# xxlong0/ESTDepth

Measured on AMD Instinct MI355X. Metric: depth frames/sec (seq_len=5, 480x640, D=64), higher is better.
Workload: dtype f32

## Files before the change

### estdepth_amd/build.py

```python
import os
import subprocess
import sys
from concurrent.futures import ThreadPoolExecutor

HERE = os.path.dirname(os.path.abspath(__file__))
ROOT = os.path.dirname(HERE)
CSRC = os.path.join(HERE, "csrc")
OUT_DIR = os.path.join(HERE, "lib")
OBJ_DIR = os.path.join(OUT_DIR, "obj" + os.environ.get("ESTD_LIB_SUFFIX", ""))
LIB = os.path.join(OUT_DIR, "libestd_hip%s.so" % os.environ.get("ESTD_LIB_SUFFIX", ""))
SOURCES = ["conv3d_mfma.hip", "conv3d_wino2.hip", "conv3d_wino3.hip", "conv3d_xout.hip", "conv3d_wino2_c16.hip", "conv2d_mfma.hip", "conv2d_wino2.hip",
           "plane_sweep.hip", "est_fusion.hip", "refine2d.hip", "conv1x1.hip", "conv2d_taps.hip", "tsdf.hip", "tsdf_raycast.hip",
           "depth_consistency.hip", "cloud_nn.hip"]
AB_SOURCES = ["conv3d_wino.hip", "conv3d_split_bf16.hip", "conv2d_wino.hip", "conv2d_split_bf16.hip", "conv3d_wino2x.hip"]
BUILD_AB = os.environ.get("ESTD_BUILD_AB", "0") == "1"
if BUILD_AB:
    SOURCES = SOURCES + AB_SOURCES
HEADERS = [os.path.join(ROOT, "include", "estd_hip.h"), os.path.join(CSRC, "estd_common.h")]
FLAGS = ["--offload-arch=gfx950", "-O3", "-std=c++17", "-fPIC",
         "-I" + os.path.join(ROOT, "include"), "-I" + CSRC] + (["-DESTD_BUILD_AB=1"] if BUILD_AB else [])
MODE_STAMP = os.path.join(OUT_DIR, ".build_mode" + os.environ.get("ESTD_LIB_SUFFIX", ""))


def _hipcc():
    for c in (os.environ.get("HIPCC"), "/opt/rocm/bin/hipcc", "hipcc"):
        if c and (os.path.isabs(c) and os.path.exists(c) or not os.path.isabs(c)):
            return c
    return "hipcc"


def _stale(target, deps):
    if not os.path.exists(target):
        return True
    t = os.path.getmtime(target)
    return any(os.path.getmtime(d) > t for d in deps)


def build(force=False, verbose=False):
    os.makedirs(OBJ_DIR, exist_ok=True)
    hipcc = _hipcc()
    mode = "ab" if BUILD_AB else "default"
    relink = (open(MODE_STAMP).read().strip() if os.path.exists(MODE_STAMP) else "default" if os.path.exists(LIB) else "") != mode
    jobs = []
    objs = []
    for src in SOURCES:
        s = os.path.join(CSRC, src)
        o = os.path.join(OBJ_DIR, src.replace(".hip", ".o"))
        objs.append(o)
        if force or _stale(o, [s] + HEADERS):
            cmd = [hipcc] + FLAGS + os.environ.get("ESTD_BUILD_DEFS", "").split() + (["-Rpass-analysis=kernel-resource-usage"] if verbose else []) + ["-c", s, "-o", o]
            jobs.append(cmd)

    def run(cmd):
        r = subprocess.run(cmd, capture_output=True, text=True)
        if r.returncode != 0:
            raise RuntimeError("hipcc failed: %s\n%s" % (" ".join(cmd), r.stderr))
        return r.stderr

    if jobs:
        with ThreadPoolExecutor(max_workers=len(jobs)) as ex:
            for log in ex.map(run, jobs):
                if verbose and log:
                    sys.stderr.write(log)
    if force or jobs or relink or _stale(LIB, objs):
        run([hipcc, "--offload-arch=gfx950", "-shared", "-fPIC"] + objs + ["-o", LIB])
    build_torch_ops(force=force or relink)
    open(MODE_STAMP, "w").write(mode)
    return LIB


TORCH_OPS_SRC = os.path.join(CSRC, "torch_ops.cpp")
TORCH_OPS_LIB = os.path.join(OUT_DIR, "libestd_torch_ops%s.so" % os.environ.get("ESTD_LIB_SUFFIX", ""))


def build_torch_ops(force=False):
    if not (force or _stale(TORCH_OPS_LIB, [TORCH_OPS_SRC, HEADERS[0], LIB])):
        return TORCH_OPS_LIB
    import torch
    from torch.utils import cpp_extension
    tlib = os.path.join(os.path.dirname(torch.__file__), "lib")
    cmd = [_hipcc(), "-O2", "-std=c++17", "-fPIC", "-shared", "-D__HIP_PLATFORM_AMD__=1", "-DUSE_ROCM=1", "-DHIPBLAS_V2",
           "-D_GLIBCXX_USE_CXX11_ABI=%d" % int(torch._C._GLIBCXX_USE_CXX11_ABI), "-I" + os.path.join(ROOT, "include")] \
        + (["-DESTD_BUILD_AB=1"] if BUILD_AB else [])
    cmd += ["-I" + p for p in cpp_extension.include_paths("cuda")]
    cmd += [TORCH_OPS_SRC, "-o", TORCH_OPS_LIB, "-L" + OUT_DIR, "-l:" + os.path.basename(LIB), "-L" + tlib,
            "-lc10", "-lc10_hip", "-ltorch_cpu", "-ltorch_hip", "-ltorch", "-Wl,-rpath,$ORIGIN", "-Wl,-rpath," + tlib]
    r = subprocess.run(cmd, capture_output=True, text=True)
    if r.returncode != 0:
        raise RuntimeError("hipcc failed: %s\n%s" % (" ".join(cmd), r.stderr[-4000:]))
    return TORCH_OPS_LIB


if __name__ == "__main__":
    print(build(force="--force" in sys.argv, verbose="--verbose" in sys.argv))
```

### estdepth_amd/csrc/conv2d_wino2.hip

```cpp
#include <hip/hip_runtime.h>
#include <stdint.h>
#include <stdlib.h>
#include <type_traits>

#include "estd_hip.h"
#include "estd_common.h"

#ifndef ESTD_C2W2ABL
#define ESTD_C2W2ABL 0
#endif

namespace {

typedef float f32x4 __attribute__((ext_vector_type(4)));
typedef float f32x2 __attribute__((ext_vector_type(2)));
typedef unsigned int u32x4 __attribute__((__vector_size__(16)));
constexpr unsigned OOB_OFFSET = 0xFFFFFF00u;

constexpr int TH = 8, TW = 16;
constexpr int TROWS = 16;
constexpr int NSTEP = 8;
#ifndef ESTD_C2W2_PFS
#define ESTD_C2W2_PFS 8
#endif
#ifndef ESTD_C2W2_WD
#define ESTD_C2W2_WD 2
#endif
#ifndef ESTD_C2W2_INLOOP
#define ESTD_C2W2_INLOOP 1
#endif
#ifndef ESTD_C2W2_INLOOP_PFS
#define ESTD_C2W2_INLOOP_PFS 4
#endif
#ifndef ESTD_C2W2_INLOOP_W0
#define ESTD_C2W2_INLOOP_W0 4
#endif
#ifndef ESTD_C2W2_SCHED
#define ESTD_C2W2_SCHED 2
#endif
#ifndef ESTD_C2W2_SPLIT
#define ESTD_C2W2_SPLIT 1
#endif
constexpr int WD = ESTD_C2W2_WD, WR = 4;

__device__ __forceinline__ float4 as_float4(u32x4 v) { float4 f; __builtin_memcpy(&f, &v, 16); return f; }
__device__ __forceinline__ u32x4 as_u32x4(float4 f) { u32x4 v; __builtin_memcpy(&v, &f, 16); return v; }
__device__ __forceinline__ float4 f4_sub(float4 a, float4 b) { return make_float4(a.x - b.x, a.y - b.y, a.z - b.z, a.w - b.w); }
__device__ __forceinline__ float4 f4_add(float4 a, float4 b) { return make_float4(a.x + b.x, a.y + b.y, a.z + b.z, a.w + b.w); }
__device__ __forceinline__ __amdgpu_buffer_rsrc_t make_rsrc(const float* base, size_t elems)
{
    return __builtin_amdgcn_make_buffer_rsrc(const_cast<float*>(base), 0, (int)(elems * 4), 0x00020000);
}
__device__ __forceinline__ void lds_barrier() { asm volatile("s_waitcnt lgkmcnt(0)\n\ts_barrier" ::: "memory"); }

template <int DIL>
__device__ __forceinline__ void wino2_rpp_nt(const estd_conv2d_desc& p, int tiles_w, int tiles_h, int total_items)
{
    constexpr int IN_H = TH + 2 * DIL, IN_W = TW + 2 * DIL;
    constexpr bool INLOOP = ESTD_C2W2_INLOOP != 0 && (DIL == 1 || ESTD_C2W2_INLOOP == 2);
    constexpr int PITCH = DIL == 1 ? IN_W + 1 : IN_W;
    constexpr int SLOT_BYTES = TROWS * PITCH * 128;
    constexpr int SH_BYTES = 4 * PITCH * 128;
    constexpr int LOADERS = IN_W * 8;
    auto lds_off = [](int row, int col, int chunk) { return (row * PITCH + col) * 128 + ((chunk ^ ((col >> 1) & 7)) << 4); };
    extern __shared__ __attribute__((aligned(16))) char smem[];

    const int tid = threadIdx.x;
    const int lane = tid & 63;
    const int wave = __builtin_amdgcn_readfirstlane(tid >> 6);
    const int rpp = wave >> 1, nt = wave & 1;
    const int g = lane >> 4, i = lane & 15;
    const int blk_rp = (i >= 4 && i < 12) ? 1 : 0;
    const int cb = i < 4 ? i : i < 12 ? i - 4 : i - 8;
    const int rp = 2 * rpp + blk_rp;
    const int row_a = DIL == 1 ? 2 * rp : (rp & 1) + 4 * (rp >> 1);
    const int col_b = DIL == 1 ? 2 * cb : (cb & 1) + 4 * (cb >> 1);
    const int H = p.H, W = p.W, Cin = p.cin, Cout = p.cout;
    const int nchunks = Cin >> 5;
    const int tiles_per_group = p.N * tiles_h * tiles_w;
    const int wlane = lane * 16 + nt * 1024;

    int u, u_end;
    {
        const int G = gridDim.x, bid = blockIdx.x;
        const int r = ((G & 7) == 0) ? (bid & 7) * (G >> 3) + (bid >> 3) : bid;
        u = (int)((long long)total_items * r / G);
        u_end = (int)((long long)total_items * (r + 1) / G);
    }
    if (u >= u_end) return;

    const size_t img_in = (size_t)H * W * Cin, img_out = (size_t)H * W * Cout;
    const bool loader = tid < LOADERS;
    const int lzx = tid >> 3, lc = tid & 7;
    const int wbase = loader ? lds_off(0, lzx, lc) : 0;

    int aoff[4];
#pragma unroll
    for (int q = 0; q < 4; ++q) aoff[q] = lds_off(rp, col_b + DIL * q, g);

    auto decode = [&](int item, int& grp, int& n, int& th0, int& tw0) {
        grp = item / tiles_per_group;
        int t = item - grp * tiles_per_group;
        const int twi = t % tiles_w; t /= tiles_w;
        const int thi = t % tiles_h; n = t / tiles_h;
        th0 = thi * TH; tw0 = twi * TW;
    };
    auto brick_offsets = [&](int th0, int tw0, unsigned (&voff)[IN_H], bool enable) {
        const int gx = tw0 - DIL + lzx;
        const bool colok = enable && loader && (unsigned)gx < (unsigned)W;
        const unsigned base = (unsigned)(gx * Cin + lc * 4) * 4u;
        const unsigned rowbytes = (unsigned)(W * Cin) * 4u;
#pragma unroll
        for (int zy = 0; zy < IN_H; ++zy) {
            const int gy = th0 - DIL + zy;
            const bool rowok = (unsigned)gy < (unsigned)H;
            voff[zy] = (colok && rowok) ? base + (unsigned)gy * rowbytes : OOB_OFFSET;
        }
    };

    int grp, n, th0, tw0;
    decode(u, grp, n, th0, tw0);
    unsigned voff[IN_H];
    brick_offsets(th0, tw0, voff, true);
    __amdgpu_buffer_rsrc_t rs_in = make_rsrc(p.in + (size_t)n * img_in, img_in);
    float4 pf[IN_H];
#pragma unroll
    for (int zy = 0; zy < IN_H; ++zy) pf[zy] = as_float4(__builtin_amdgcn_raw_buffer_load_b128(rs_in, voff[zy], 0, 0));

    const size_t wgrp_elems = (size_t)nchunks * NSTEP * 4 * 2 * 256;
    float4 bq[WR][4];
    {
        const __amdgpu_buffer_rsrc_t rs_w0 = make_rsrc(p.w_wino + (size_t)grp * wgrp_elems, wgrp_elems);
#pragma unroll
        for (int s = 0; s < WD; ++s)
#pragma unroll
            for (int sw = 0; sw < 4; ++sw) bq[s][sw] = as_float4(__builtin_amdgcn_raw_buffer_load_b128(rs_w0, wlane, (s * 4 + sw) * 2048, 0));
    }
    const float floor_b = p.relu_before_residual ? 0.f : ESTD_NO_FLOOR;
    const float floor_a = p.relu_after_residual ? 0.f : ESTD_NO_FLOOR;

    int k = 0;
    if (INLOOP) {
        if (loader && !(ESTD_C2W2ABL & 2)) {
#pragma unroll
            for (int w = 0; w < 4; ++w) {
                const int a = DIL == 1 ? 2 * w : (w & 1) + 4 * (w >> 1);
                const float4 d0 = pf[a], d1 = pf[a + DIL], d2 = pf[a + 2 * DIL], d3 = pf[a + 3 * DIL];
                *reinterpret_cast<float4*>(smem + wbase + (0 * 4 + w) * PITCH * 128) = f4_sub(d0, d2);
                *reinterpret_cast<float4*>(smem + wbase + (1 * 4 + w) * PITCH * 128) = f4_add(d1, d2);
                *reinterpret_cast<float4*>(smem + wbase + (2 * 4 + w) * PITCH * 128) = f4_sub(d2, d1);
                *reinterpret_cast<float4*>(smem + wbase + (3 * 4 + w) * PITCH * 128) = f4_sub(d1, d3);
            }
        }
    }
    while (true) {
        const __amdgpu_buffer_rsrc_t rs_w = make_rsrc(p.w_wino + (size_t)grp * wgrp_elems, wgrp_elems);
        const int cbase = grp * 32 + nt * 16 + 4 * g;
        const float4 sc4 = *reinterpret_cast<const float4*>(p.scale + cbase), sh4 = *reinterpret_cast<const float4*>(p.shift + cbase);
        f32x4 acc[4][4];

        const bool has_next_item = (u + 1 < u_end);
        int ngrp = grp, nn_ = n, nth0 = th0, ntw0 = tw0;
        if (has_next_item) decode(u + 1, ngrp, nn_, nth0, ntw0);
        const __amdgpu_buffer_rsrc_t rs_wni = make_rsrc(p.w_wino + (size_t)ngrp * wgrp_elems, wgrp_elems);

        auto write_rows = [&](char* slot, int w0, int w1) {
            if (loader && !(ESTD_C2W2ABL & 2)) {
#pragma unroll
                for (int w = 0; w < 4; ++w) {
                    if (w < w0 || w >= w1) continue;
                    const int a = DIL == 1 ? 2 * w : (w & 1) + 4 * (w >> 1);
                    const float4 d0 = pf[a], d1 = pf[a + DIL], d2 = pf[a + 2 * DIL], d3 = pf[a + 3 * DIL];
                    *reinterpret_cast<float4*>(slot + wbase + (0 * 4 + w) * PITCH * 128) = f4_sub(d0, d2);
                    *reinterpret_cast<float4*>(slot + wbase + (1 * 4 + w) * PITCH * 128) = f4_add(d1, d2);
                    *reinterpret_cast<float4*>(slot + wbase + (2 * 4 + w) * PITCH * 128) = f4_sub(d2, d1);
                    *reinterpret_cast<float4*>(slot + wbase + (3 * 4 + w) * PITCH * 128) = f4_sub(d1, d3);
                }
            }
        };
        auto write_row_sh = [&](char* slot, int w, int sh_) {
            if (loader && !(ESTD_C2W2ABL & 2)) {
                const int a = DIL == 1 ? 2 * w : (w & 1) + 4 * (w >> 1);
                const float4 d0 = pf[a], d1 = pf[a + DIL], d2 = pf[a + 2 * DIL], d3 = pf[a + 3 * DIL];
                const float4 v = sh_ == 0 ? f4_sub(d0, d2) : sh_ == 1 ? f4_add(d1, d2) : sh_ == 2 ? f4_sub(d2, d1) : f4_sub(d1, d3);
                *reinterpret_cast<float4*>(slot + wbase + (sh_ * 4 + w) * PITCH * 128) = v;
            }
        };
        auto chunk_body = [&](auto first_c, const int c) {
            constexpr bool FIRST = decltype(first_c)::value;
            const int sb = (k & 1) * SLOT_BYTES;
            char* slot = smem + sb;
            if (!INLOOP) write_rows(slot, 0, 4);
            lds_barrier();

            const bool last_chunk = (c + 1 == nchunks);
            int pf_soff = (c + 1) * 128;
            if (last_chunk) {
                brick_offsets(nth0, ntw0, voff, has_next_item);
                if (nn_ != n) rs_in = make_rsrc(p.in + (size_t)nn_ * img_in, img_in);
                pf_soff = 0;
            }
            const int wbase_q = c * NSTEP * 4;
            const __amdgpu_buffer_rsrc_t rs_wx = last_chunk ? rs_wni : rs_w;
            const int wnext_q = last_chunk ? 0 : wbase_q + NSTEP * 4;

            int ao[4];
#pragma unroll
            for (int q = 0; q < 4; ++q) ao[q] = aoff[q] + sb;
            auto load_rows = [&](int st, float4 (&Rr)[4]) {
#pragma unroll
                for (int q = 0; q < 4; ++q)
                    Rr[q] = *reinterpret_cast<const float4*>(smem + ((st & 1) ? (ao[q] ^ 64) : ao[q]) + (st >> 1) * SH_BYTES);
            };
            auto xform2 = [&](const float4 (&Rr)[4], int h, f32x2 (&o)[4]) {
                f32x2 r[4];
#pragma unroll
                for (int q = 0; q < 4; ++q) r[q] = h == 0 ? (f32x2){Rr[q].x, Rr[q].y} : (f32x2){Rr[q].z, Rr[q].w};
                if (ESTD_C2W2ABL & 128) { o[0] = r[0]; o[1] = r[1]; o[2] = r[2]; o[3] = r[3]; }
                else { o[0] = r[0] - r[2]; o[1] = r[1] + r[2]; o[2] = r[2] - r[1]; o[3] = r[1] - r[3]; }
            };
            f32x2 T[2][4];
            float4 R[4];
            load_rows(0, R);
            xform2(R, 0, T[0]);
            xform2(R, 1, T[1]);
            load_rows(1, R);
            __builtin_amdgcn_sched_barrier(0);

#pragma clang loop unroll(full)
            for (int st = 0; st < NSTEP; ++st) {
                const int sh = st >> 1;
                f32x2 Tn[2][4];
                if (ESTD_C2W2_SCHED == 2) {
                    constexpr int PFS = INLOOP ? ESTD_C2W2_INLOOP_PFS : ESTD_C2W2_PFS;
                    const int r0 = PFS != 8 ? (st < PFS ? st * IN_H / PFS : IN_H) : DIL == 1 ? (st == 0 ? 0 : st + 1) : (3 * st + 1) / 2;
                    const int r1 = PFS != 8 ? (st < PFS ? (st + 1) * IN_H / PFS : IN_H)
                                            : DIL == 1 ? ((st == 0 || st == NSTEP - 1) ? r0 + 2 : r0 + 1) : (3 * (st + 1) + 1) / 2;
                    const bool wr = INLOOP && st >= ESTD_C2W2_INLOOP_W0 && (!last_chunk || has_next_item);
                    constexpr int WN = NSTEP - ESTD_C2W2_INLOOP_W0;
                    static_assert(!INLOOP || WN == 4, "quarter schedule: one row pair of the next chunk per step");
#pragma unroll
                    for (int h = 0; h < 2; ++h) {
#pragma unroll
                        for (int e = 0; e < 2; ++e) {
                            const int qk = 2 * h + e;
                            if (!(ESTD_C2W2ABL & 8)) {
                                const int tgt = st + WD;
                                bq[tgt % WR][qk] = tgt < NSTEP
                                    ? as_float4(__builtin_amdgcn_raw_buffer_load_b128(rs_w, wlane, (wbase_q + tgt * 4 + qk) * 2048, 0))
                                    : as_float4(__builtin_amdgcn_raw_buffer_load_b128(rs_wx, wlane, (wnext_q + (tgt - NSTEP) * 4 + qk) * 2048, 0));
                            }
#pragma unroll
                            for (int r = r0 + (r1 - r0) * qk / 4; r < r0 + (r1 - r0) * (qk + 1) / 4; ++r)
                                pf[r] = as_float4(__builtin_amdgcn_raw_buffer_load_b128(rs_in, voff[r], pf_soff, 0));
                            if (wr) write_row_sh(smem + (((k + 1) & 1) * SLOT_BYTES), st - ESTD_C2W2_INLOOP_W0, qk);
                            __builtin_amdgcn_sched_barrier(0);
#pragma unroll
                            for (int sw = 0; sw < 4; ++sw) {
                                const float4 b4 = bq[(ESTD_C2W2ABL & 8) ? 0 : st % WR][sw];
                                const float b = h == 0 ? (e == 0 ? b4.x : b4.y) : (e == 0 ? b4.z : b4.w);
                                const bool first_product = FIRST && (st & 1) == 0 && h == 0 && e == 0;
                                const f32x4 c_in = first_product ? (f32x4){0.f, 0.f, 0.f, 0.f} : acc[sh][sw];
                                acc[sh][sw] = __builtin_amdgcn_mfma_f32_16x16x4f32(b, T[h][sw][e], c_in, 0, 0, 0);
                            }
                            if (e == 1 && st + 1 < NSTEP) xform2(R, h, Tn[h]);
                            __builtin_amdgcn_sched_barrier(0);
                        }
                    }
                } else {
                if (!(ESTD_C2W2ABL & 8)) {
                    const int tgt = st + WD;
#pragma unroll
                    for (int sw = 0; sw < 4; ++sw)
                        bq[tgt % WR][sw] = tgt < NSTEP
                            ? as_float4(__builtin_amdgcn_raw_buffer_load_b128(rs_w, wlane, (wbase_q + tgt * 4 + sw) * 2048, 0))
                            : as_float4(__builtin_amdgcn_raw_buffer_load_b128(rs_wx, wlane, (wnext_q + (tgt - NSTEP) * 4 + sw) * 2048, 0));
                }
                {
                    constexpr int PFS = INLOOP ? ESTD_C2W2_INLOOP_PFS : ESTD_C2W2_PFS;
                    const int r0 = PFS != 8 ? (st < PFS ? st * IN_H / PFS : IN_H) : DIL == 1 ? (st == 0 ? 0 : st + 1) : (3 * st + 1) / 2;
                    const int r1 = PFS != 8 ? (st < PFS ? (st + 1) * IN_H / PFS : IN_H)
                                            : DIL == 1 ? ((st == 0 || st == NSTEP - 1) ? r0 + 2 : r0 + 1) : (3 * (st + 1) + 1) / 2;
#pragma unroll
                    for (int r = r0; r < r1; ++r) pf[r] = as_float4(__builtin_amdgcn_raw_buffer_load_b128(rs_in, voff[r], pf_soff, 0));
                }
                if (INLOOP && st >= ESTD_C2W2_INLOOP_W0 && (!last_chunk || has_next_item)) {
                    constexpr int WN = NSTEP - ESTD_C2W2_INLOOP_W0;
                    const int i0 = (st - ESTD_C2W2_INLOOP_W0) * 4 / WN, i1 = (st - ESTD_C2W2_INLOOP_W0 + 1) * 4 / WN;
                    write_rows(smem + (((k + 1) & 1) * SLOT_BYTES), i0, i1);
                }
                if (!ESTD_C2W2_SCHED) __builtin_amdgcn_sched_barrier(0);
#pragma unroll
                for (int h = 0; h < 2; ++h) {
#pragma unroll
                    for (int e = 0; e < 2; ++e)
#pragma unroll
                        for (int sw = 0; sw < 4; ++sw) {
                            const float4 b4 = bq[(ESTD_C2W2ABL & 8) ? 0 : st % WR][sw];
                            const float b = h == 0 ? (e == 0 ? b4.x : b4.y) : (e == 0 ? b4.z : b4.w);
                            const bool first_product = FIRST && (st & 1) == 0 && h == 0 && e == 0;
                            const f32x4 c_in = first_product ? (f32x4){0.f, 0.f, 0.f, 0.f} : acc[sh][sw];
                            acc[sh][sw] = __builtin_amdgcn_mfma_f32_16x16x4f32(b, T[h][sw][e], c_in, 0, 0, 0);
                        }
                    if (st + 1 < NSTEP) xform2(R, h, Tn[h]);
                }
                }
                if (st + 2 < NSTEP) load_rows(st + 2, R);
                if (ESTD_C2W2_SCHED == 2) {
                    __builtin_amdgcn_sched_group_barrier(0x100, 4, 0);
                } else if (ESTD_C2W2_SCHED) {
#pragma unroll
                    for (int i = 0; i < 8; ++i) {
                        __builtin_amdgcn_sched_group_barrier(0x008, 2, 0);
                        __builtin_amdgcn_sched_group_barrier(0x020, 1, 0);
                        __builtin_amdgcn_sched_group_barrier(0x200, 1, 0);
                        __builtin_amdgcn_sched_group_barrier(0x002, 4, 0);
                    }
                    __builtin_amdgcn_sched_group_barrier(0x100, 4, 0);
                } else {
#pragma unroll
                    for (int h = 0; h < 2; ++h) {
                        __builtin_amdgcn_sched_group_barrier(0x008, 8, 0);
                        __builtin_amdgcn_sched_group_barrier(0x002, 4, 0);
                    }
                    __builtin_amdgcn_sched_group_barrier(0x100, 4, 0);
                }
                if (st + 1 < NSTEP) {
#pragma unroll
                    for (int h = 0; h < 2; ++h)
#pragma unroll
                        for (int sw = 0; sw < 4; ++sw) T[h][sw] = Tn[h][sw];
                }
                __builtin_amdgcn_sched_barrier(0);
            }
        };
        chunk_body(std::true_type{}, 0);
        ++k;
        for (int c = 1; c < nchunks; ++c, ++k) chunk_body(std::false_type{}, c);

        auto epilogue = [&](auto has_res_c) {
            constexpr bool HAS_RES = decltype(has_res_c)::value;
            const __amdgpu_buffer_rsrc_t rs_out = make_rsrc(p.out + (size_t)n * img_out, img_out);
            const __amdgpu_buffer_rsrc_t rs_res = make_rsrc((HAS_RES ? p.residual : p.out) + (size_t)n * img_out, img_out);
            const float floor_1 = HAS_RES ? floor_b : fmaxf(floor_b, floor_a);
            unsigned eo[2][2];
#pragma unroll
            for (int r = 0; r < 2; ++r)
#pragma unroll
                for (int j = 0; j < 2; ++j) {
                    const int y = th0 + row_a + DIL * r, x = tw0 + col_b + DIL * j;
                    eo[r][j] = (y < H && x < W) ? (unsigned)((y * W + x) * Cout + cbase) * 4u : OOB_OFFSET;
                }
            float4 res[2][2];
            if (HAS_RES) {
#pragma unroll
                for (int r = 0; r < 2; ++r)
#pragma unroll
                    for (int j = 0; j < 2; ++j) res[r][j] = as_float4(__builtin_amdgcn_raw_buffer_load_b128(rs_res, eo[r][j], 0, 0));
            }
            f32x4 z[4][2];
#pragma unroll
            for (int s = 0; s < 4; ++s) {
                z[s][0] = acc[s][0] + acc[s][1] + acc[s][2];
                z[s][1] = acc[s][1] - acc[s][2] - acc[s][3];
            }
#pragma unroll
            for (int r = 0; r < 2; ++r)
#pragma unroll
                for (int j = 0; j < 2; ++j) {
                    const f32x4 yv = r == 0 ? z[0][j] + z[1][j] + z[2][j] : z[1][j] - z[2][j] - z[3][j];
                    float4 v;
                    v.x = fmaxf(fmaf(yv[0], sc4.x, sh4.x), floor_1); v.y = fmaxf(fmaf(yv[1], sc4.y, sh4.y), floor_1);
                    v.z = fmaxf(fmaf(yv[2], sc4.z, sh4.z), floor_1); v.w = fmaxf(fmaf(yv[3], sc4.w, sh4.w), floor_1);
                    if (HAS_RES) {
                        v.x = fmaxf(v.x + res[r][j].x, floor_a); v.y = fmaxf(v.y + res[r][j].y, floor_a);
                        v.z = fmaxf(v.z + res[r][j].z, floor_a); v.w = fmaxf(v.w + res[r][j].w, floor_a);
                    }
                    if (ESTD_C2W2ABL & 1) asm volatile("" :: "v"(v.x), "v"(v.w));
                    else __builtin_amdgcn_raw_buffer_store_b128(as_u32x4(v), rs_out, eo[r][j], 0, 0);
                }
        };
        if (p.residual) epilogue(std::true_type{}); else epilogue(std::false_type{});

        if (!has_next_item) break;
        ++u;
        grp = ngrp; n = nn_; th0 = nth0; tw0 = ntw0;
    }
}

template <int DIL, bool WIDE>
__device__ __forceinline__ void wino2_split(const estd_conv2d_desc& p, int tiles_w, int tiles_h, int total_items)
{
    constexpr int TH_ = WIDE ? TH / 2 : TH;
    constexpr int NP = TH_ / 2;
    constexpr int IN_H = TH_ + 2 * DIL, IN_W = TW + 2 * DIL;
    constexpr bool INLOOP = ESTD_C2W2_INLOOP != 0 && (DIL == 1 || ESTD_C2W2_INLOOP == 2);
    constexpr int PITCH = DIL == 1 ? IN_W + 1 : IN_W;
    constexpr int ROW_BYTES = PITCH * 128;
    constexpr int SLOT_BYTES = 4 * NP * ROW_BYTES;
    constexpr int SH_BYTES = NP * ROW_BYTES;
    constexpr int LOADERS = IN_W * 8;
    constexpr int NQ = 4;
    auto lds_off = [](int row, int col, int chunk) { return row * ROW_BYTES + col * 128 + ((chunk ^ ((col >> 1) & 7)) << 4); };
    extern __shared__ __attribute__((aligned(16))) char smem[];

    const int tid = threadIdx.x;
    const int lane = tid & 63;
    const int wave = __builtin_amdgcn_readfirstlane(tid >> 6);
    const int shp = wave & 1, sel = wave >> 1;
    const int g = lane >> 4, i = lane & 15;
    const int blk_rp = (i >= 4 && i < 12) ? 1 : 0;
    const int cb = i < 4 ? i : i < 12 ? i - 4 : i - 8;
    const int rp = (WIDE ? 0 : 2 * sel) + blk_rp;
    const int row_a = DIL == 1 ? 2 * rp : (rp & 1) + 4 * (rp >> 1);
    const int col_b = DIL == 1 ? 2 * cb : (cb & 1) + 4 * (cb >> 1);
    const int H = p.H, W = p.W, Cin = p.cin, Cout = p.cout;
    const int nchunks = Cin >> 5;
    const int tiles_per_group = p.N * tiles_h * tiles_w;
    const int wlane = lane * 16;
    const int srec = shp * 16;

    int u, u_end;
    {
        const int G = gridDim.x, bid = blockIdx.x;
        const int r = ((G & 7) == 0) ? (bid & 7) * (G >> 3) + (bid >> 3) : bid;
        u = (int)((long long)total_items * r / G);
        u_end = (int)((long long)total_items * (r + 1) / G);
    }
    if (u >= u_end) return;

    const size_t img_in = (size_t)H * W * Cin, img_out = (size_t)H * W * Cout;
    const bool loader = tid < LOADERS;
    const int lzx = tid >> 3, lc = tid & 7;
    const int wbase = loader ? lds_off(0, lzx, lc) : 0;

    int aoff[4];
#pragma unroll
    for (int q = 0; q < 4; ++q) aoff[q] = lds_off(rp, col_b + DIL * q, g);

    auto decode = [&](int item, int& grp, int& n, int& th0, int& tw0) {
        grp = item / tiles_per_group;
        int t = item - grp * tiles_per_group;
        const int twi = t % tiles_w; t /= tiles_w;
        const int thi = t % tiles_h; n = t / tiles_h;
        th0 = thi * TH_; tw0 = twi * TW;
    };
    auto brick_offsets = [&](int th0, int tw0, unsigned (&voff)[IN_H], bool enable) {
        const int gx = tw0 - DIL + lzx;
        const bool colok = enable && loader && (unsigned)gx < (unsigned)W;
        const unsigned base = (unsigned)(gx * Cin + lc * 4) * 4u;
        const unsigned rowbytes = (unsigned)(W * Cin) * 4u;
#pragma unroll
        for (int zy = 0; zy < IN_H; ++zy) {
            const int gy = th0 - DIL + zy;
            const bool rowok = (unsigned)gy < (unsigned)H;
            voff[zy] = (colok && rowok) ? base + (unsigned)gy * rowbytes : OOB_OFFSET;
        }
    };

    int grp, n, th0, tw0;
    decode(u, grp, n, th0, tw0);
    unsigned voff[IN_H];
    brick_offsets(th0, tw0, voff, true);
    __amdgpu_buffer_rsrc_t rs_in = make_rsrc(p.in + (size_t)n * img_in, img_in);
    float4 pf[IN_H];
#pragma unroll
    for (int zy = 0; zy < IN_H; ++zy) pf[zy] = as_float4(__builtin_amdgcn_raw_buffer_load_b128(rs_in, voff[zy], 0, 0));

    const size_t wgrp_elems = (size_t)nchunks * NSTEP * 4 * 2 * 256;
    auto wgrp_rsrc = [&](int grp_) { return make_rsrc(p.w_wino + (size_t)(WIDE ? 2 * grp_ + sel : grp_) * wgrp_elems, wgrp_elems); };
    float4 bw[2][4][2];
    {
        const __amdgpu_buffer_rsrc_t rs_w0 = wgrp_rsrc(grp);
#pragma unroll
        for (int sw = 0; sw < 4; ++sw)
#pragma unroll
            for (int t = 0; t < 2; ++t) bw[0][sw][t] = as_float4(__builtin_amdgcn_raw_buffer_load_b128(rs_w0, wlane, (srec + sw) * 2048 + t * 1024, 0));
    }
    const float floor_b = p.relu_before_residual ? 0.f : ESTD_NO_FLOOR;
    const float floor_a = p.relu_after_residual ? 0.f : ESTD_NO_FLOOR;

    auto write_row_sh = [&](char* slot, int w, int sh_) {
        if (loader && !(ESTD_C2W2ABL & 2)) {
            const int a = DIL == 1 ? 2 * w : (w & 1) + 4 * (w >> 1);
            const float4 d0 = pf[a], d1 = pf[a + DIL], d2 = pf[a + 2 * DIL], d3 = pf[a + 3 * DIL];
            const float4 v = sh_ == 0 ? f4_sub(d0, d2) : sh_ == 1 ? f4_add(d1, d2) : sh_ == 2 ? f4_sub(d2, d1) : f4_sub(d1, d3);
            *reinterpret_cast<float4*>(slot + wbase + (sh_ * NP + w) * ROW_BYTES) = v;
        }
    };
    auto write_rows = [&](char* slot) {
#pragma unroll
        for (int w = 0; w < NP; ++w)
#pragma unroll
            for (int s = 0; s < 4; ++s) write_row_sh(slot, w, s);
    };

    int k = 0;
    if (INLOOP) write_rows(smem);
    while (true) {
        const __amdgpu_buffer_rsrc_t rs_w = wgrp_rsrc(grp);
        const int cbase = (WIDE ? 64 * grp + 32 * sel : 32 * grp) + 4 * g;
        f32x4 acc[2][4][2];

        const bool has_next_item = (u + 1 < u_end);
        int ngrp = grp, nn_ = n, nth0 = th0, ntw0 = tw0;
        if (has_next_item) decode(u + 1, ngrp, nn_, nth0, ntw0);
        const __amdgpu_buffer_rsrc_t rs_wni = wgrp_rsrc(ngrp);

        auto chunk_body = [&](auto first_c, const int c) {
            constexpr bool FIRST = decltype(first_c)::value;
            const int sb = (k & 1) * SLOT_BYTES;
            char* slot = smem + sb;
            if (!INLOOP) write_rows(slot);
            lds_barrier();

            const bool last_chunk = (c + 1 == nchunks);
            int pf_soff = (c + 1) * 128;
            if (last_chunk) {
                brick_offsets(nth0, ntw0, voff, has_next_item);
                if (nn_ != n) rs_in = make_rsrc(p.in + (size_t)nn_ * img_in, img_in);
                pf_soff = 0;
            }
            const int wrec = c * NSTEP * 4 + srec;
            const __amdgpu_buffer_rsrc_t rs_wx = last_chunk ? rs_wni : rs_w;
            const int wrec_x = (last_chunk ? 0 : (c + 1) * NSTEP * 4) + srec;

            int ao[4];
#pragma unroll
            for (int q = 0; q < 4; ++q) ao[q] = aoff[q] + sb + 2 * shp * SH_BYTES;
            auto load_rows = [&](int L, float4 (&Rr)[4]) {
#pragma unroll
                for (int q = 0; q < 4; ++q)
                    Rr[q] = *reinterpret_cast<const float4*>(smem + ((L & 1) ? (ao[q] ^ 64) : ao[q]) + (L >> 1) * SH_BYTES);
            };
            auto xform2 = [&](const float4 (&Rr)[4], int h, f32x2 (&o)[4]) {
                f32x2 r[4];
#pragma unroll
                for (int q = 0; q < 4; ++q) r[q] = h == 0 ? (f32x2){Rr[q].x, Rr[q].y} : (f32x2){Rr[q].z, Rr[q].w};
                if (ESTD_C2W2ABL & 128) { o[0] = r[0]; o[1] = r[1]; o[2] = r[2]; o[3] = r[3]; }
                else { o[0] = r[0] - r[2]; o[1] = r[1] + r[2]; o[2] = r[2] - r[1]; o[3] = r[1] - r[3]; }
            };
            f32x2 T[2][4];
            float4 R[4];
            load_rows(0, R);
            xform2(R, 0, T[0]);
            xform2(R, 1, T[1]);
            load_rows(1, R);
            __builtin_amdgcn_sched_barrier(0);

#pragma clang loop unroll(full)
            for (int L = 0; L < NQ; ++L) {
                const int sl = L >> 1;
                f32x2 Tn[2][4];
#pragma unroll
                for (int q = 0; q < 4; ++q) {
                    const int j = NQ * L + q;
                    if (!(ESTD_C2W2ABL & 8)) {
#pragma unroll
                        for (int t = 0; t < 2; ++t)
                            bw[(L + 1) & 1][q][t] = L + 1 < NQ
                                ? as_float4(__builtin_amdgcn_raw_buffer_load_b128(rs_w, wlane, (wrec + (L + 1) * 4 + q) * 2048 + t * 1024, 0))
                                : as_float4(__builtin_amdgcn_raw_buffer_load_b128(rs_wx, wlane, (wrec_x + q) * 2048 + t * 1024, 0));
                    }
                    constexpr int NJ = INLOOP ? 2 * 4 : NQ * 4;
#pragma unroll
                    for (int r = IN_H * j / NJ; r < (j < NJ ? IN_H * (j + 1) / NJ : 0); ++r)
                        pf[r] = as_float4(__builtin_amdgcn_raw_buffer_load_b128(rs_in, voff[r], pf_soff, 0));
                    if (INLOOP && L >= 2 && (!last_chunk || has_next_item)) {
                        char* nslot = smem + ((k + 1) & 1) * SLOT_BYTES;
                        const int jw = j - 8;
                        if (WIDE) write_row_sh(nslot, jw >> 2, jw & 3);
                        else { write_row_sh(nslot, jw >> 1, 2 * (jw & 1)); write_row_sh(nslot, jw >> 1, 2 * (jw & 1) + 1); }
                    }
                    __builtin_amdgcn_sched_barrier(0);
#pragma unroll
                    for (int h = 0; h < 2; ++h)
#pragma unroll
                        for (int e = 0; e < 2; ++e)
#pragma unroll
                            for (int t = 0; t < 2; ++t) {
                                const float4 b4 = bw[(ESTD_C2W2ABL & 8) ? 0 : L & 1][q][t];
                                const float b = h == 0 ? (e == 0 ? b4.x : b4.y) : (e == 0 ? b4.z : b4.w);
                                const bool first_product = FIRST && (L & 1) == 0 && h == 0 && e == 0;
                                const f32x4 c_in = first_product ? (f32x4){0.f, 0.f, 0.f, 0.f} : acc[sl][q][t];
                                acc[sl][q][t] = __builtin_amdgcn_mfma_f32_16x16x4f32(b, T[h][q][e], c_in, 0, 0, 0);
                            }
                    if ((q & 1) && L + 1 < NQ) xform2(R, q >> 1, Tn[q >> 1]);
                    __builtin_amdgcn_sched_barrier(0);
                }
                if (L + 2 < NQ) load_rows(L + 2, R);
                __builtin_amdgcn_sched_group_barrier(0x100, 4, 0);
                if (L + 1 < NQ) {
#pragma unroll
                    for (int h = 0; h < 2; ++h)
#pragma unroll
                        for (int sw = 0; sw < 4; ++sw) T[h][sw] = Tn[h][sw];
                }
                __builtin_amdgcn_sched_barrier(0);
            }
        };
        chunk_body(std::true_type{}, 0);
        ++k;
        for (int c = 1; c < nchunks; ++c, ++k) chunk_body(std::false_type{}, c);

        const float4 sc4[2] = {*reinterpret_cast<const float4*>(p.scale + cbase), *reinterpret_cast<const float4*>(p.scale + cbase + 16)};
        const float4 sh4[2] = {*reinterpret_cast<const float4*>(p.shift + cbase), *reinterpret_cast<const float4*>(p.shift + cbase + 16)};
        f32x4 z[2][2][2];
#pragma unroll
        for (int sl = 0; sl < 2; ++sl)
#pragma unroll
            for (int t = 0; t < 2; ++t) {
                z[sl][0][t] = acc[sl][0][t] + acc[sl][1][t] + acc[sl][2][t];
                z[sl][1][t] = acc[sl][1][t] - acc[sl][2][t] - acc[sl][3][t];
            }
        char* xb = WIDE ? smem + 2 * SLOT_BYTES : smem + ((k - 1) & 1) * SLOT_BYTES;
        if (!WIDE) lds_barrier();
#pragma unroll
        for (int v = 0; v < 4; ++v)
            *reinterpret_cast<f32x4*>(xb + wave * 4096 + (v * 64 + lane) * 16) = shp == 0 ? z[1][v >> 1][v & 1] : z[0][v >> 1][v & 1];
        lds_barrier();
        f32x4 zo[2][2];
#pragma unroll
        for (int v = 0; v < 4; ++v) zo[v >> 1][v & 1] = *reinterpret_cast<const f32x4*>(xb + (wave ^ 1) * 4096 + (v * 64 + lane) * 16);

        auto epilogue = [&](auto has_res_c) {
            constexpr bool HAS_RES = decltype(has_res_c)::value;
            const __amdgpu_buffer_rsrc_t rs_out = make_rsrc(p.out + (size_t)n * img_out, img_out);
            const __amdgpu_buffer_rsrc_t rs_res = make_rsrc((HAS_RES ? p.residual : p.out) + (size_t)n * img_out, img_out);
            const float floor_1 = HAS_RES ? floor_b : fmaxf(floor_b, floor_a);
            const int y = th0 + row_a + DIL * shp;
            unsigned eo[2][2];
#pragma unroll
            for (int j = 0; j < 2; ++j)
#pragma unroll
                for (int t = 0; t < 2; ++t) {
                    const int x = tw0 + col_b + DIL * j;
                    eo[j][t] = (y < H && x < W) ? (unsigned)((y * W + x) * Cout + cbase + 16 * t) * 4u : OOB_OFFSET;
                }
            float4 res[2][2];
            if (HAS_RES) {
#pragma unroll
                for (int j = 0; j < 2; ++j)
#pragma unroll
                    for (int t = 0; t < 2; ++t) res[j][t] = as_float4(__builtin_amdgcn_raw_buffer_load_b128(rs_res, eo[j][t], 0, 0));
            }
#pragma unroll
            for (int j = 0; j < 2; ++j)
#pragma unroll
                for (int t = 0; t < 2; ++t) {
                    const f32x4 yv = shp == 0 ? z[0][j][t] + z[1][j][t] + zo[j][t] : zo[j][t] - z[0][j][t] - z[1][j][t];
                    float4 v;
                    v.x = fmaxf(fmaf(yv[0], sc4[t].x, sh4[t].x), floor_1); v.y = fmaxf(fmaf(yv[1], sc4[t].y, sh4[t].y), floor_1);
                    v.z = fmaxf(fmaf(yv[2], sc4[t].z, sh4[t].z), floor_1); v.w = fmaxf(fmaf(yv[3], sc4[t].w, sh4[t].w), floor_1);
                    if (HAS_RES) {
                        v.x = fmaxf(v.x + res[j][t].x, floor_a); v.y = fmaxf(v.y + res[j][t].y, floor_a);
                        v.z = fmaxf(v.z + res[j][t].z, floor_a); v.w = fmaxf(v.w + res[j][t].w, floor_a);
                    }
                    if (ESTD_C2W2ABL & 1) asm volatile("" :: "v"(v.x), "v"(v.w));
                    else __builtin_amdgcn_raw_buffer_store_b128(as_u32x4(v), rs_out, eo[j][t], 0, 0);
                }
        };
        if (p.residual) epilogue(std::true_type{}); else epilogue(std::false_type{});

        if (!has_next_item) break;
        ++u;
        grp = ngrp; n = nn_; th0 = nth0; tw0 = ntw0;
    }
}

template <int DIL>
__global__ __launch_bounds__(256, 2) void conv2d_wino2_kernel(const estd_conv2d_desc p, int tiles_w, int tiles_h, int total_items)
{
#if ESTD_C2W2_SPLIT
    if ((p.cout & 63) == 0) { wino2_split<DIL, true>(p, tiles_w, tiles_h, total_items); return; }
#endif
#if ESTD_C2W2_SPLIT == 2
    wino2_split<DIL, false>(p, tiles_w, tiles_h, total_items);
#else
    wino2_rpp_nt<DIL>(p, tiles_w, tiles_h, total_items);
#endif
}

}

extern "C" int estd_conv2d_k3_wino2(const estd_conv2d_desc* dp, estd_stream_t s)
{
    if (!dp) return ESTD_ERR_ARG;
    const estd_conv2d_desc& d = *dp;
    if (d.N <= 0 || d.H <= 0 || d.W <= 0 || !d.in || !d.w_wino || !d.scale || !d.shift || !d.out) return ESTD_ERR_ARG;
    if (d.cin < 32 || (d.cin & 31) || d.cout < 32 || (d.cout & 31)) return ESTD_ERR_ARG;
    if (d.dilation != 1 && d.dilation != 2) return ESTD_ERR_UNSUPPORTED;
    const long long widest = (long long)d.H * d.W * (d.cin > d.cout ? d.cin : d.cout) * 4;
    if (widest >= 0x7fffff00LL) return ESTD_ERR_UNSUPPORTED;
    const bool wide = ESTD_C2W2_SPLIT != 0 && (d.cout & 63) == 0;
    const int th = wide ? TH / 2 : TH;
    const int tiles_w = (d.W + TW - 1) / TW, tiles_h = (d.H + th - 1) / th;
    const int groups = d.cout / (wide ? 64 : 32);
    const long long total = (long long)groups * d.N * tiles_h * tiles_w;
    if (total > 0x7fffffffLL) return ESTD_ERR_ARG;
    const int slots = estd_persistent_wgs(2);
    int grid = total < slots ? (int)total : slots;
    if (grid >= 8) grid &= ~7;
    const size_t rows = wide ? TROWS / 2 : TROWS, xchg = wide ? 16384 : 0;
    if (d.dilation == 1) {
        const size_t lds = 2 * rows * (TW + 3) * 128 + xchg;
        estd_allow_dynamic_lds<conv2d_wino2_kernel<1>>(2 * TROWS * (TW + 3) * 128);
        hipLaunchKernelGGL(conv2d_wino2_kernel<1>, dim3(grid), dim3(256), lds, estd_stream(s), d, tiles_w, tiles_h, (int)total);
    } else {
        const size_t lds = 2 * rows * (TW + 4) * 128 + xchg;
        estd_allow_dynamic_lds<conv2d_wino2_kernel<2>>(2 * TROWS * (TW + 4) * 128);
        hipLaunchKernelGGL(conv2d_wino2_kernel<2>, dim3(grid), dim3(256), lds, estd_stream(s), d, tiles_w, tiles_h, (int)total);
    }
    return ESTD_LAUNCH_CHECK();
}
```

Baseline: 198.3.

## Add quad-wave Winograd F(2,3) conv2d path splitting row transforms across waves

Adds a new wino2_quad kernel path, made the default via ESTD_C2W2_SPLIT=3, for 64-wide output groups. Each of the four waves handles one vertical Winograd transform component (sh) and accumulates partial products over all channel chunks. The per-wave results are then exchanged through a larger LDS buffer to finish the output transform. The build also produces a variant library that keeps the old split kernel for A/B comparison. The aim is to spread the input-transform and MFMA work differently and reduce per-wave redundant transforms, at the cost of more LDS exchange space and a barrier-heavy epilogue.

```diff
diff --git a/estdepth_amd/build.py b/estdepth_amd/build.py
--- a/estdepth_amd/build.py
+++ b/estdepth_amd/build.py
@@ -20,6 +20,9 @@
 FLAGS = ["--offload-arch=gfx950", "-O3", "-std=c++17", "-fPIC",
          "-I" + os.path.join(ROOT, "include"), "-I" + CSRC] + (["-DESTD_BUILD_AB=1"] if BUILD_AB else [])
 MODE_STAMP = os.path.join(OUT_DIR, ".build_mode" + os.environ.get("ESTD_LIB_SUFFIX", ""))
+VARIANTS = {"_split1": ("conv2d_wino2.hip", ["-DESTD_C2W2_SPLIT=1"])}
+if os.environ.get("ESTD_LIB_SUFFIX") or os.environ.get("ESTD_BUILD_DEFS"):
+    VARIANTS = {}
 
 
 def _hipcc():
@@ -50,6 +53,12 @@
         if force or _stale(o, [s] + HEADERS):
             cmd = [hipcc] + FLAGS + os.environ.get("ESTD_BUILD_DEFS", "").split() + (["-Rpass-analysis=kernel-resource-usage"] if verbose else []) + ["-c", s, "-o", o]
             jobs.append(cmd)
+    vlibs = []
+    for suffix, (src, defs) in VARIANTS.items():
+        s, o = os.path.join(CSRC, src), os.path.join(OBJ_DIR, src.replace(".hip", suffix + ".o"))
+        vlibs.append((os.path.join(OUT_DIR, "libestd_hip%s.so" % suffix), [o if x == os.path.join(OBJ_DIR, src.replace(".hip", ".o")) else x for x in objs]))
+        if force or _stale(o, [s] + HEADERS):
+            jobs.append([hipcc] + FLAGS + defs + ["-c", s, "-o", o])
 
     def run(cmd):
         r = subprocess.run(cmd, capture_output=True, text=True)
@@ -64,6 +73,9 @@
                     sys.stderr.write(log)
     if force or jobs or relink or _stale(LIB, objs):
         run([hipcc, "--offload-arch=gfx950", "-shared", "-fPIC"] + objs + ["-o", LIB])
+    for vlib, vobjs in vlibs:
+        if force or jobs or relink or _stale(vlib, vobjs):
+            run([hipcc, "--offload-arch=gfx950", "-shared", "-fPIC"] + vobjs + ["-o", vlib])
     build_torch_ops(force=force or relink)
     open(MODE_STAMP, "w").write(mode)
     return LIB
diff --git a/estdepth_amd/csrc/conv2d_wino2.hip b/estdepth_amd/csrc/conv2d_wino2.hip
--- a/estdepth_amd/csrc/conv2d_wino2.hip
+++ b/estdepth_amd/csrc/conv2d_wino2.hip
@@ -39,7 +39,7 @@
 #define ESTD_C2W2_SCHED 2
 #endif
 #ifndef ESTD_C2W2_SPLIT
-#define ESTD_C2W2_SPLIT 1
+#define ESTD_C2W2_SPLIT 3
 #endif
 constexpr int WD = ESTD_C2W2_WD, WR = 4;
 
@@ -669,9 +669,289 @@
 }
 
 template <int DIL>
+__device__ __forceinline__ void wino2_quad(const estd_conv2d_desc& p, int tiles_w, int tiles_h, int total_items)
+{
+    constexpr int TH_ = TH / 2;
+    constexpr int NP = TH_ / 2;
+    constexpr int IN_H = TH_ + 2 * DIL, IN_W = TW + 2 * DIL;
+    constexpr bool INLOOP = ESTD_C2W2_INLOOP != 0 && (DIL == 1 || ESTD_C2W2_INLOOP == 2);
+    constexpr int PITCH = DIL == 1 ? IN_W + 1 : IN_W;
+    constexpr int ROW_BYTES = PITCH * 128;
+    constexpr int SLOT_BYTES = 4 * NP * ROW_BYTES;
+    constexpr int SH_BYTES = NP * ROW_BYTES;
+    constexpr int LOADERS = IN_W * 8;
+    constexpr int NQ = 2;
+    constexpr int XW_BYTES = 8 * 64 * 16;
+    auto lds_off = [](int row, int col, int chunk) { return row * ROW_BYTES + col * 128 + ((chunk ^ ((col >> 1) & 7)) << 4); };
+    extern __shared__ __attribute__((aligned(16))) char smem[];
+
+    const int tid = threadIdx.x;
+    const int lane = tid & 63;
+    const int wave = __builtin_amdgcn_readfirstlane(tid >> 6);
+    const int er = wave & 1, eh = wave >> 1;
+    const int g = lane >> 4, i = lane & 15;
+    const int rp = (i >= 4 && i < 12) ? 1 : 0;
+    const int cb = i < 4 ? i : i < 12 ? i - 4 : i - 8;
+    const int row_a = DIL == 1 ? 2 * rp : rp;
+    const int col_b = DIL == 1 ? 2 * cb : (cb & 1) + 4 * (cb >> 1);
+    const int H = p.H, W = p.W, Cin = p.cin, Cout = p.cout;
+    const int nchunks = Cin >> 5;
+    const int tiles_per_group = p.N * tiles_h * tiles_w;
+    const int wlane = lane * 16;
+    const int srec = wave * 8;
+
+    int u, u_end;
+    {
+        const int G = gridDim.x, bid = blockIdx.x;
+        const int r = ((G & 7) == 0) ? (bid & 7) * (G >> 3) + (bid >> 3) : bid;
+        u = (int)((long long)total_items * r / G);
+        u_end = (int)((long long)total_items * (r + 1) / G);
+    }
+    if (u >= u_end) return;
+
+    const size_t img_in = (size_t)H * W * Cin, img_out = (size_t)H * W * Cout;
+    const bool loader = tid < LOADERS;
+    const int lzx = tid >> 3, lc = tid & 7;
+    const int wbase = loader ? lds_off(0, lzx, lc) : 0;
+
+    int aoff[4];
+#pragma unroll
+    for (int q = 0; q < 4; ++q) aoff[q] = lds_off(rp, col_b + DIL * q, g) + wave * SH_BYTES;
+
+    auto decode = [&](int item, int& grp, int& n, int& th0, int& tw0) {
+        grp = item / tiles_per_group;
+        int t = item - grp * tiles_per_group;
+        const int twi = t % tiles_w; t /= tiles_w;
+        const int thi = t % tiles_h; n = t / tiles_h;
+        th0 = thi * TH_; tw0 = twi * TW;
+    };
+    auto brick_offsets = [&](int th0, int tw0, unsigned (&voff)[IN_H], bool enable) {
+        const int gx = tw0 - DIL + lzx;
+        const bool colok = enable && loader && (unsigned)gx < (unsigned)W;
+        const unsigned base = (unsigned)(gx * Cin + lc * 4) * 4u;
+        const unsigned rowbytes = (unsigned)(W * Cin) * 4u;
+#pragma unroll
+        for (int zy = 0; zy < IN_H; ++zy) {
+            const int gy = th0 - DIL + zy;
+            const bool rowok = (unsigned)gy < (unsigned)H;
+            voff[zy] = (colok && rowok) ? base + (unsigned)gy * rowbytes : OOB_OFFSET;
+        }
+    };
+
+    int grp, n, th0, tw0;
+    decode(u, grp, n, th0, tw0);
+    unsigned voff[IN_H];
+    brick_offsets(th0, tw0, voff, true);
+    __amdgpu_buffer_rsrc_t rs_in = make_rsrc(p.in + (size_t)n * img_in, img_in);
+    float4 pf[IN_H];
+#pragma unroll
+    for (int zy = 0; zy < IN_H; ++zy) pf[zy] = as_float4(__builtin_amdgcn_raw_buffer_load_b128(rs_in, voff[zy], 0, 0));
+
+    const size_t wgrp_elems = (size_t)nchunks * NSTEP * 4 * 2 * 256;
+    const int wgrp_bytes = (int)(wgrp_elems * 4);
+    auto wgrp_rsrc = [&](int grp_) { return make_rsrc(p.w_wino + (size_t)(2 * grp_) * wgrp_elems, 2 * wgrp_elems); };
+    auto wtile = [&](int t) { return (t >> 1) * wgrp_bytes + (t & 1) * 1024; };
+    float4 bw[4][4];
+    {
+        const __amdgpu_buffer_rsrc_t rs_w0 = wgrp_rsrc(grp);
+#pragma unroll
+        for (int sw = 0; sw < 3; ++sw)
+#pragma unroll
+            for (int t = 0; t < 4; ++t) bw[sw][t] = as_float4(__builtin_amdgcn_raw_buffer_load_b128(rs_w0, wlane, (srec + sw) * 2048 + wtile(t), 0));
+    }
+    const float floor_b = p.relu_before_residual ? 0.f : ESTD_NO_FLOOR;
+    const float floor_a = p.relu_after_residual ? 0.f : ESTD_NO_FLOOR;
+
+    auto write_row_sh = [&](char* slot, int w, int sh_) {
+        if (loader && !(ESTD_C2W2ABL & 2)) {
+            const int a = DIL == 1 ? 2 * w : w;
+            const float4 d0 = pf[a], d1 = pf[a + DIL], d2 = pf[a + 2 * DIL], d3 = pf[a + 3 * DIL];
+            const float4 v = sh_ == 0 ? f4_sub(d0, d2) : sh_ == 1 ? f4_add(d1, d2) : sh_ == 2 ? f4_sub(d2, d1) : f4_sub(d1, d3);
+            *reinterpret_cast<float4*>(slot + wbase + (sh_ * NP + w) * ROW_BYTES) = v;
+        }
+    };
+    auto write_rows = [&](char* slot) {
+#pragma unroll
+        for (int w = 0; w < NP; ++w)
+#pragma unroll
+            for (int s = 0; s < 4; ++s) write_row_sh(slot, w, s);
+    };
+
+    int k = 0;
+    if (INLOOP) write_rows(smem);
+    while (true) {
+        const __amdgpu_buffer_rsrc_t rs_w = wgrp_rsrc(grp);
+        const int cbase = 64 * grp + 32 * eh + 4 * g;
+        f32x4 acc[4][4];
+
+        const bool has_next_item = (u + 1 < u_end);
+        int ngrp = grp, nn_ = n, nth0 = th0, ntw0 = tw0;
+        if (has_next_item) decode(u + 1, ngrp, nn_, nth0, ntw0);
+        const __amdgpu_buffer_rsrc_t rs_wni = wgrp_rsrc(ngrp);
+
+        auto chunk_body = [&](auto first_c, const int c) {
+            constexpr bool FIRST = decltype(first_c)::value;
+            const int sb = (k & 1) * SLOT_BYTES;
+            char* slot = smem + sb;
+            if (!INLOOP) write_rows(slot);
+            lds_barrier();
+
+            const bool last_chunk = (c + 1 == nchunks);
+            int pf_soff = (c + 1) * 128;
+            if (last_chunk) {
+                brick_offsets(nth0, ntw0, voff, has_next_item);
+                if (nn_ != n) rs_in = make_rsrc(p.in + (size_t)nn_ * img_in, img_in);
+                pf_soff = 0;
+            }
+            const int wrec = c * NSTEP * 4 + srec;
+            const __amdgpu_buffer_rsrc_t rs_wx = last_chunk ? rs_wni : rs_w;
+            const int wrec_x = (last_chunk ? 0 : (c + 1) * NSTEP * 4) + srec;
+
+            int ao[4];
+#pragma unroll
+            for (int q = 0; q < 4; ++q) ao[q] = aoff[q] + sb;
+            auto load_rows = [&](int L, float4 (&Rr)[4]) {
+#pragma unroll
+                for (int q = 0; q < 4; ++q) Rr[q] = *reinterpret_cast<const float4*>(smem + (L ? (ao[q] ^ 64) : ao[q]));
+            };
+            auto xform2 = [&](const float4 (&Rr)[4], int h, f32x2 (&o)[4]) {
+                f32x2 r[4];
+#pragma unroll
+                for (int q = 0; q < 4; ++q) r[q] = h == 0 ? (f32x2){Rr[q].x, Rr[q].y} : (f32x2){Rr[q].z, Rr[q].w};
+                if (ESTD_C2W2ABL & 128) { o[0] = r[0]; o[1] = r[1]; o[2] = r[2]; o[3] = r[3]; }
+                else { o[0] = r[0] - r[2]; o[1] = r[1] + r[2]; o[2] = r[2] - r[1]; o[3] = r[1] - r[3]; }
+            };
+            f32x2 T[2][4];
+            float4 R[4];
+            load_rows(0, R);
+            xform2(R, 0, T[0]);
+            xform2(R, 1, T[1]);
+            load_rows(1, R);
+            __builtin_amdgcn_sched_barrier(0);
+
+#pragma clang loop unroll(full)
+            for (int L = 0; L < NQ; ++L) {
+                f32x2 Tn[2][4];
+#pragma unroll
+                for (int q = 0; q < 4; ++q) {
+                    const int j = 4 * L + q;
+                    if (!(ESTD_C2W2ABL & 8)) {
+                        const int sw_ = (q + 3) & 3;
+#pragma unroll
+                        for (int t = 0; t < 4; ++t)
+                            bw[sw_][t] = q == 0 ? as_float4(__builtin_amdgcn_raw_buffer_load_b128(rs_w, wlane, (wrec + L * 4 + sw_) * 2048 + wtile(t), 0))
+                                       : L + 1 < NQ ? as_float4(__builtin_amdgcn_raw_buffer_load_b128(rs_w, wlane, (wrec + (L + 1) * 4 + sw_) * 2048 + wtile(t), 0))
+                                       : as_float4(__builtin_amdgcn_raw_buffer_load_b128(rs_wx, wlane, (wrec_x + sw_) * 2048 + wtile(t), 0));
+                    }
+                    constexpr int NJ = INLOOP ? 4 : NQ * 4;
+#pragma unroll
+                    for (int r = IN_H * j / NJ; r < (j < NJ ? IN_H * (j + 1) / NJ : 0); ++r)
+                        pf[r] = as_float4(__builtin_amdgcn_raw_buffer_load_b128(rs_in, voff[r], pf_soff, 0));
+                    if (INLOOP && L == 1 && (!last_chunk || has_next_item)) {
+                        char* nslot = smem + ((k + 1) & 1) * SLOT_BYTES;
+                        write_row_sh(nslot, q >> 1, 2 * (q & 1));
+                        write_row_sh(nslot, q >> 1, 2 * (q & 1) + 1);
+                    }
+                    __builtin_amdgcn_sched_barrier(0);
+#pragma unroll
+                    for (int h = 0; h < 2; ++h)
+#pragma unroll
+                        for (int e = 0; e < 2; ++e)
+#pragma unroll
+                            for (int t = 0; t < 4; ++t) {
+                                const float4 b4 = bw[(ESTD_C2W2ABL & 8) ? 0 : q][(ESTD_C2W2ABL & 8) ? 0 : t];
+                                const float b = h == 0 ? (e == 0 ? b4.x : b4.y) : (e == 0 ? b4.z : b4.w);
+                                const bool first_product = FIRST && L == 0 && h == 0 && e == 0;
+                                const f32x4 c_in = first_product ? (f32x4){0.f, 0.f, 0.f, 0.f} : acc[q][t];
+                                acc[q][t] = __builtin_amdgcn_mfma_f32_16x16x4f32(b, T[h][q][e], c_in, 0, 0, 0);
+                            }
+                    if ((q & 1) && L + 1 < NQ) xform2(R, q >> 1, Tn[q >> 1]);
+                    __builtin_amdgcn_sched_barrier(0);
+                }
+                if (L + 1 < NQ) {
+#pragma unroll
+                    for (int h = 0; h < 2; ++h)
+#pragma unroll
+                        for (int sw = 0; sw < 4; ++sw) T[h][sw] = Tn[h][sw];
+                }
+                __builtin_amdgcn_sched_barrier(0);
+            }
+        };
+        chunk_body(std::true_type{}, 0);
+        ++k;
+        for (int c = 1; c < nchunks; ++c, ++k) chunk_body(std::false_type{}, c);
+
+        const float4 sc4[2] = {*reinterpret_cast<const float4*>(p.scale + cbase), *reinterpret_cast<const float4*>(p.scale + cbase + 16)};
+        const float4 sh4[2] = {*reinterpret_cast<const float4*>(p.shift + cbase), *reinterpret_cast<const float4*>(p.shift + cbase + 16)};
+        char* xb = smem + 2 * SLOT_BYTES;
+#pragma unroll
+        for (int t = 0; t < 4; ++t) {
+            const f32x4 z0 = acc[0][t] + acc[1][t] + acc[2][t];
+            const f32x4 z1 = acc[1][t] - acc[2][t] - acc[3][t];
+            *reinterpret_cast<f32x4*>(xb + wave * XW_BYTES + ((0 * 4 + t) * 64 + lane) * 16) = z0;
+            *reinterpret_cast<f32x4*>(xb + wave * XW_BYTES + ((1 * 4 + t) * 64 + lane) * 16) = z1;
+        }
+        lds_barrier();
+        f32x4 zs[3][2][2];
+#pragma unroll
+        for (int a = 0; a < 3; ++a)
+#pragma unroll
+            for (int j = 0; j < 2; ++j)
+#pragma unroll
+                for (int t = 0; t < 2; ++t)
+                    zs[a][j][t] = *reinterpret_cast<const f32x4*>(xb + (er + a) * XW_BYTES + ((j * 4 + 2 * eh + t) * 64 + lane) * 16);
+
+        auto epilogue = [&](auto has_res_c) {
+            constexpr bool HAS_RES = decltype(has_res_c)::value;
+            const __amdgpu_buffer_rsrc_t rs_out = make_rsrc(p.out + (size_t)n * img_out, img_out);
+            const __amdgpu_buffer_rsrc_t rs_res = make_rsrc((HAS_RES ? p.residual : p.out) + (size_t)n * img_out, img_out);
+            const float floor_1 = HAS_RES ? floor_b : fmaxf(floor_b, floor_a);
+            const int y = th0 + row_a + DIL * er;
+            unsigned eo[2][2];
+#pragma unroll
+            for (int j = 0; j < 2; ++j)
+#pragma unroll
+                for (int t = 0; t < 2; ++t) {
+                    const int x = tw0 + col_b + DIL * j;
+                    eo[j][t] = (y < H && x < W) ? (unsigned)((y * W + x) * Cout + cbase + 16 * t) * 4u : OOB_OFFSET;
+                }
+            float4 res[2][2];
+            if (HAS_RES) {
+#pragma unroll
+                for (int j = 0; j < 2; ++j)
+#pragma unroll
+                    for (int t = 0; t < 2; ++t) res[j][t] = as_float4(__builtin_amdgcn_raw_buffer_load_b128(rs_res, eo[j][t], 0, 0));
+            }
+#pragma unroll
+            for (int j = 0; j < 2; ++j)
+#pragma unroll
+                for (int t = 0; t < 2; ++t) {
+                    const f32x4 yv = er == 0 ? zs[0][j][t] + zs[1][j][t] + zs[2][j][t] : zs[0][j][t] - zs[1][j][t] - zs[2][j][t];
+                    float4 v;
+                    v.x = fmaxf(fmaf(yv[0], sc4[t].x, sh4[t].x), floor_1); v.y = fmaxf(fmaf(yv[1], sc4[t].y, sh4[t].y), floor_1);
+                    v.z = fmaxf(fmaf(yv[2], sc4[t].z, sh4[t].z), floor_1); v.w = fmaxf(fmaf(yv[3], sc4[t].w, sh4[t].w), floor_1);
+                    if (HAS_RES) {
+                        v.x = fmaxf(v.x + res[j][t].x, floor_a); v.y = fmaxf(v.y + res[j][t].y, floor_a);
+                        v.z = fmaxf(v.z + res[j][t].z, floor_a); v.w = fmaxf(v.w + res[j][t].w, floor_a);
+                    }
+                    if (ESTD_C2W2ABL & 1) asm volatile("" :: "v"(v.x), "v"(v.w));
+                    else __builtin_amdgcn_raw_buffer_store_b128(as_u32x4(v), rs_out, eo[j][t], 0, 0);
+                }
+        };
+        if (p.residual) epilogue(std::true_type{}); else epilogue(std::false_type{});
+
+        if (!has_next_item) break;
+        ++u;
+        grp = ngrp; n = nn_; th0 = nth0; tw0 = ntw0;
+    }
+}
+
+template <int DIL>
 __global__ __launch_bounds__(256, 2) void conv2d_wino2_kernel(const estd_conv2d_desc p, int tiles_w, int tiles_h, int total_items)
 {
-#if ESTD_C2W2_SPLIT
+#if ESTD_C2W2_SPLIT == 3
+    if ((p.cout & 63) == 0) { wino2_quad<DIL>(p, tiles_w, tiles_h, total_items); return; }
+#elif ESTD_C2W2_SPLIT
     if ((p.cout & 63) == 0) { wino2_split<DIL, true>(p, tiles_w, tiles_h, total_items); return; }
 #endif
 #if ESTD_C2W2_SPLIT == 2
@@ -701,7 +981,7 @@
     const int slots = estd_persistent_wgs(2);
     int grid = total < slots ? (int)total : slots;
     if (grid >= 8) grid &= ~7;
-    const size_t rows = wide ? TROWS / 2 : TROWS, xchg = wide ? 16384 : 0;
+    const size_t rows = wide ? TROWS / 2 : TROWS, xchg = wide ? (ESTD_C2W2_SPLIT == 3 ? 32768 : 16384) : 0;
     if (d.dilation == 1) {
         const size_t lds = 2 * rows * (TW + 3) * 128 + xchg;
         estd_allow_dynamic_lds<conv2d_wino2_kernel<1>>(2 * TROWS * (TW + 3) * 128);
```

Result: slower. 195.2 (-1.5%).
